# BradenDKelly/MetropolisMonteCarlo

Measured on AMD Instinct MI355X. Metric: MC trial moves/sec (whole node), SPC/E NVT full Ewald fp64, higher is better.
Workload: dtype f64

## Files before the change

### metropolismontecarlo_amd/csrc/mmc_wave.hpp

```cpp
#pragma once
#include "mmc_fast.hpp"
#include "mmc_propose.hpp"

#ifndef WV_WAVES
#define WV_WAVES 4
#endif
#ifndef WV_OCC
#define WV_OCC 5
#endif
#ifndef WV_OCC_WOLF
#define WV_OCC_WOLF 4
#endif
#ifndef WV_MWAVES
#define WV_MWAVES WV_WAVES
#endif
#ifndef WV_LIST
#define WV_LIST 640
#endif
#ifndef WV_PF
#define WV_PF 6
#endif
#define MMC_CQ_PAD (4 * 64 * (2 * WV_PF + 2))
#ifndef WV_TPF
#define WV_TPF 3
#endif

typedef uint16_t wv_list_t;
#define MMC_WAVE_MAX_MOL 65535
template <int NW, bool PT = true> struct WaveSharedT {
    alignas(16) double qtab[MMC_QQ_TABLE_DOUBLES];
    cplx ptab[NW][2][3][3][MMC_NKTAB];
    wv_list_t list[NW][WV_LIST];
    alignas(16) double pvw[NW][12];
    alignas(16) double outw[NW][8];
    __device__ __forceinline__ double *sum6w(int wv) { return reinterpret_cast<double *>(&ptab[wv][0][0][0][0]); }
};
template <int NW> struct WaveSharedT<NW, false> {
    alignas(16) double qtab[MMC_QQ_TABLE_DOUBLES];
    alignas(16) double sum6[NW][24];
    wv_list_t list[NW][WV_LIST];
    alignas(16) double pvw[NW][12];
    alignas(16) double outw[NW][8];
    __device__ __forceinline__ double *sum6w(int wv) { return sum6[wv]; }
};
typedef WaveSharedT<WV_WAVES> WaveShared;

#ifdef WV_STAMPS
#define WV_NSTAMP 8
__device__ unsigned long long g_wv_stamps[65536 * WV_NSTAMP];
#define WV_STAMP(i)                                                                              \
    do {                                                                                         \
        asm volatile("s_waitcnt vmcnt(0) lgkmcnt(0)" ::: "memory");                              \
        if (lane == 0 && unit < 65536)                                                           \
            g_wv_stamps[unit * WV_NSTAMP + (i)] = __builtin_amdgcn_s_memtime();                  \
    } while (0)
#else
#define WV_STAMP(i)
#endif

__device__ __forceinline__ void wave_sync()
{
    __builtin_amdgcn_fence(__ATOMIC_RELEASE, "wavefront");
    __builtin_amdgcn_wave_barrier();
    __builtin_amdgcn_fence(__ATOMIC_ACQUIRE, "wavefront");
}

__device__ __forceinline__ double dpp_quad_swap_f64(double v)
{
    const long long b = __double_as_longlong(v);
    const unsigned lo = (unsigned)__builtin_amdgcn_update_dpp(0, (int)b, 0xB1, 0xf, 0xf, true),
                   hi = (unsigned)__builtin_amdgcn_update_dpp(0, (int)(b >> 32), 0xB1, 0xf, 0xf, true);
    return __longlong_as_double((long long)(((unsigned long long)hi << 32) | lo));
}
__device__ __forceinline__ void wave_sum6_add(double v0, double v1, double v2, double v3, double v4,
                                              double v5, double *out, double *scratch, int lane)
{
    const bool odd = (lane & 1) != 0;
    double p0 = (odd ? v1 : v0) + dpp_quad_swap_f64(odd ? v0 : v1);
    double p1 = (odd ? v3 : v2) + dpp_quad_swap_f64(odd ? v2 : v3);
    double p2 = (odd ? v5 : v4) + dpp_quad_swap_f64(odd ? v4 : v5);
    p0 += dpp_row_shr_f64<2>(p0); p1 += dpp_row_shr_f64<2>(p1); p2 += dpp_row_shr_f64<2>(p2);
    p0 += dpp_row_shr_f64<4>(p0); p1 += dpp_row_shr_f64<4>(p1); p2 += dpp_row_shr_f64<4>(p2);
    p0 += dpp_row_shr_f64<8>(p0); p1 += dpp_row_shr_f64<8>(p1); p2 += dpp_row_shr_f64<8>(p2);
    if ((lane & 14) == 14) {
        double *dst = scratch + 4 * (lane & 1) + (lane >> 4);
        dst[0] = p0; dst[8] = p1; dst[16] = p2;
    }
    __builtin_amdgcn_fence(__ATOMIC_RELEASE, "wavefront");
    __builtin_amdgcn_wave_barrier();
    __builtin_amdgcn_fence(__ATOMIC_ACQUIRE, "wavefront");
    if (lane < 6) {
        const double *r = scratch + 4 * lane;
        out[lane] += ((r[0] + r[1]) + r[2]) + r[3];
    }
}
__device__ __forceinline__ void wave_sum4_add(double v0, double v1, double v4, double v5, double *out,
                                              double *scratch, int lane)
{
    const bool odd = (lane & 1) != 0;
    double p0 = (odd ? v1 : v0) + dpp_quad_swap_f64(odd ? v0 : v1);
    double p1 = (odd ? v5 : v4) + dpp_quad_swap_f64(odd ? v4 : v5);
    p0 += dpp_row_shr_f64<2>(p0); p1 += dpp_row_shr_f64<2>(p1);
    p0 += dpp_row_shr_f64<4>(p0); p1 += dpp_row_shr_f64<4>(p1);
    p0 += dpp_row_shr_f64<8>(p0); p1 += dpp_row_shr_f64<8>(p1);
    if ((lane & 14) == 14) {
        double *dst = scratch + 4 * (lane & 1) + (lane >> 4);
        dst[0] = p0; dst[8] = p1;
    }
    __builtin_amdgcn_fence(__ATOMIC_RELEASE, "wavefront");
    __builtin_amdgcn_wave_barrier();
    __builtin_amdgcn_fence(__ATOMIC_ACQUIRE, "wavefront");
    if (lane < 4) {
        const double *r = scratch + 4 * lane;
        out[lane < 2 ? lane : lane + 2] += ((r[0] + r[1]) + r[2]) + r[3];
    }
}
__device__ __forceinline__ void wave_sum1_store(double v, double *out, double *scratch, int lane)
{
    v += dpp_row_shr_f64<1>(v);
    v += dpp_row_shr_f64<2>(v);
    v += dpp_row_shr_f64<4>(v);
    v += dpp_row_shr_f64<8>(v);
    if ((lane & 15) == 15)
        scratch[lane >> 4] = v;
    __builtin_amdgcn_fence(__ATOMIC_RELEASE, "wavefront");
    __builtin_amdgcn_wave_barrier();
    __builtin_amdgcn_fence(__ATOMIC_ACQUIRE, "wavefront");
    if (lane == 0)
        *out = ((scratch[0] + scratch[1]) + scratch[2]) + scratch[3];
}

__device__ __forceinline__ int lane_i32(int v, int src)
{
    return __builtin_amdgcn_readlane(v, src);
}

__device__ __forceinline__ double uniform_f64(double v)
{
    const long long b = __double_as_longlong(v);
    unsigned lo, hi;
    asm volatile("v_readfirstlane_b32 %0, %1" : "=s"(lo) : "v"((int)b));
    asm volatile("v_readfirstlane_b32 %0, %1" : "=s"(hi) : "v"((int)(b >> 32)));
    return __longlong_as_double((long long)(((unsigned long long)hi << 32) | lo));
}

__device__ __forceinline__ double lane_f64(double v, int src)
{
    const long long b = __double_as_longlong(v);
    const unsigned lo = (unsigned)__builtin_amdgcn_readlane((int)b, src);
    const unsigned hi = (unsigned)__builtin_amdgcn_readlane((int)(b >> 32), src);
    return __longlong_as_double((long long)(((unsigned long long)hi << 32) | lo));
}

__device__ __forceinline__ void phase_row_moderate(double x, double L, cplx *row )
{
    double sn, cs;
    sincos_moderate(MMC_TWOPI * x / L, sn, cs);
    const cplx e1 = { cs, sn }, one = { 1.0, 0.0 };
    row[5] = one;
    row[6] = e1;
    row[4] = c_conj(e1);
    cplx p = e1;
#pragma unroll
    for (int k = 2; k <= 5; k++) {
        p = c_mul(p, e1);
        row[5 + k] = p;
        row[5 - k] = c_conj(p);
    }
}

__device__ __forceinline__ int wave_decide(const double *outw, bool ov_old, bool ov_new,
                                           const DecideConsts *__restrict__ dc, long long step, int r,
                                           int scur, int lane, double *delta_out = nullptr, bool store_flags = true,
                                           bool flip_s = true)
{
    const double delta = mmc_move_delta(outw, ov_old, ov_new, dc->factor);
    if (delta_out)
        *delta_out = delta;
    const double x = delta / dc->temperature;
    const double u = mmc_metropolis_uniform(ChainKey{ dc->seed, dc->replica0 + (uint32_t)r }, (uint64_t)step);
    bool met;
    if (x < 0.0) met = true;
    else if (1.0 - x > u + 1e-9) met = true;
    else if ((1.0 + x) * u > 1.0 + 1e-9) met = false;
    else met = exp(-x) > u;
    const int acc = (met && !(ov_old || ov_new)) ? 1 : 0;
    if (store_flags && lane == 0)
        dc->flags[r] = (uint8_t)(acc | ((scur ^ (flip_s ? acc : 0)) << 1));
    return acc;
}

__device__ __forceinline__ int wave_ticket(unsigned *queue, unsigned base, int n_waves, int lane)
{
    unsigned t = 0;
    if (lane == 0)
        t = atomicAdd(queue, 1u);
    return n_waves + (int)(__builtin_amdgcn_readfirstlane(t) - base);
}

template <bool SUBST, bool IMG, bool MULTI = false, bool WOLF = false>
__global__ __launch_bounds__(WV_MWAVES * 64)
__attribute__((amdgpu_waves_per_eu(WOLF ? WV_OCC_WOLF : WV_OCC, WOLF ? WV_OCC_WOLF : WV_OCC))) void k_move_eval_wave(
    BatchView bv, double *rec, const double *__restrict__ qq_tab,
    const int32_t *__restrict__ kpack, FastConsts fc, const MoveRec *__restrict__ cur,
    const MoveRec *__restrict__ prev, PartOut *out, int n_parts, PairParams pp, int r_base,
    int n_units, const uint8_t *flagv, unsigned stamp, const DecideConsts *__restrict__ dc, long long dec_step,
    int n_sub_arg, int slot0, unsigned *queue, unsigned queue_base)
{
    const int n_sub = MULTI ? n_sub_arg : 1;
    __shared__ __align__(16) WaveSharedT<WV_MWAVES, !WOLF> sm;
    const int tid = threadIdx.x, lane0 = tid & 63;
    const int wv = __builtin_amdgcn_readfirstlane(tid >> 6);

    for (int k = tid; k < MMC_QQ_TABLE_DOUBLES; k += WV_MWAVES * 64)
        sm.qtab[k] = qq_tab[k];
    __syncthreads();

    const int n_mol = bv.n_mol, nkv = bv.nkvecs;
    const double box = bv.box;
    const BoxConsts bc = box_consts(box);
    const int np = WOLF ? n_parts : (n_parts == 1) ? 1 : n_parts - 1;
    const int plen = (n_mol + np - 1) / np;
    const bool same_gate = pp.lj_gate_sq == pp.qq_gate_sq;
    const double inv_box = uniform_f64(1.0 / box);
    uint32_t gate_q;
    asm volatile("v_readfirstlane_b32 %0, %1" : "=s"(gate_q) : "v"(com_quant_gate(fmax(pp.lj_gate_sq, pp.qq_gate_sq), box)));
    wv_list_t *const list = sm.list[wv];
    const double *const pvw = sm.pvw[wv];

    for (int unit = blockIdx.x * WV_MWAVES + wv; unit < n_units;
         unit = MULTI && queue ? wave_ticket(queue, queue_base, gridDim.x * WV_MWAVES, lane0)
                               : unit + gridDim.x * WV_MWAVES) {
        int lane = lane0;
        if (!MULTI)
            asm volatile("" : "+v"(lane));
        int rl = unit, part = 0;
        if (n_parts != 1) {
            rl = unit / n_parts;
            part = unit - rl * n_parts;
        }
        const int r = r_base + rl;
        const bool do_pairs = WOLF ? true : (n_parts == 1) || (part < n_parts - 1);
        const bool do_recip = WOLF ? false : (n_parts == 1) || (part == n_parts - 1);
        const int j_begin = do_pairs ? min(part * plen, n_mol) : 0;
        const int j_end = do_pairs ? min(j_begin + plen, n_mol) : 0;
        double *const myrec = rec + (int64_t)r * n_mol * MMC_RSTRIDE;

        int flags_carry = -1;
        double e_sum = 0.0;
        unsigned acc_mask = 0, ovl_mask = 0, kind_mask = 0;
      for (int sub = 0; sub < n_sub; sub++) {
        if (MULTI) {
            lane = lane0;
            asm volatile("" : "+v"(lane));
        }
        const MoveRec *cur_s = cur, *prev_s = prev;
        if (n_sub > 1) {
            const int sl = (slot0 + sub) % dc->ring_slots, slp = (slot0 + sub + dc->ring_slots - 1) % dc->ring_slots;
            cur_s = dc->ring + (int64_t)sl * dc->ring_stride;
            if (sub > 0)
                prev_s = dc->ring + (int64_t)slp * dc->ring_stride;
        }
        WV_STAMP(0);
        const double *mvp = reinterpret_cast<const double *>(cur_s + r);
        double w = 0.0;
        if (lane < MV_Q_NEW)
            w = mvp[lane];
        WV_STAMP(1);
        const int gflag = flags_carry >= 0 ? flags_carry : (flagv ? __builtin_amdgcn_readfirstlane((int)flagv[r]) : -1);
        const long long hdr = __double_as_longlong(w);
        const int i0 = lane_i32((int)hdr, 0) - 1;
        const int flags = gflag >= 0 ? gflag : lane_i32((int)(hdr >> 32), 0);
        const bool commit = prev_s && (flags & 1);
        const int scur = (flags >> 1) & 1;

        int pend = -1;
        if (commit) {
            const double *pvp = reinterpret_cast<const double *>(prev_s + r);
            double pw = 0.0;
            if (lane < 9) pw = pvp[MV_AT_NEW + lane];
            else if (lane < 12) pw = pvp[MV_COM_NEW + lane - 9];
            else if (lane == 12) pw = pvp[0];
            else if (lane < 17) pw = pvp[MV_Q_NEW + lane - 13];
            pend = lane_i32((int)__double_as_longlong(pw), 12) - 1;
            if (lane < 12)
                sm.pvw[wv][lane] = pw;
            if (part == 0 && lane < 12) {
                myrec[(int64_t)pend * MMC_RSTRIDE + lane] = pw;
                if (lane < 9) {
                    const int a = lane / 3, d = lane % 3;
                    (d == 0 ? bv.ax : d == 1 ? bv.ay : bv.az)[r * bv.atom_stride + 3 * pend + a] = pw;
                } else {
                    const int d = lane - 9;
                    (d == 0 ? bv.comx : d == 1 ? bv.comy : bv.comz)[r * bv.mol_stride + pend] = pw;
                    comq_store(bv, r, pend, d, pw, inv_box);
                }
            }
            if (bv.quat) {
                const double q0 = wave_pick(pw, 13), q1 = wave_pick(pw, 14),
                             q2 = wave_pick(pw, 15), q3 = wave_pick(pw, 16);
                if (part == 0 && lane >= 13 && lane < 17)
                    quat_commit(bv, r, pend, lane - 13, pw, q0 * q0 + q1 * q1 + q2 * q2 + q3 * q3 > 0.25);
            }
            wave_sync();
            if (WOLF && !SUBST)
                asm volatile("s_waitcnt vmcnt(0)" ::: "memory");
        }

#define WV_CQ_BASE (bv.comq + (int64_t)r * 3 * bv.cq_stride)
#define WV_PART_DST (out + (int64_t)r * n_parts + part)
        auto decide_here = [&](bool o0, bool o1) -> int {
            if (!dc)
                return 0;
            if (n_sub <= 1)
                return wave_decide(sm.outw[wv], o0, o1, dc, dec_step, r, scur, lane, nullptr, true, !WOLF);
            double delta;
            const bool last = sub + 1 == n_sub;
            const int acc = wave_decide(sm.outw[wv], o0, o1, dc, dec_step + sub, r, scur, lane, &delta, last, !WOLF);
            if (acc) {
                e_sum += delta;
                acc_mask |= 1u << sub;
            }
            if (o0 || o1)
                ovl_mask |= 1u << sub;
            kind_mask |= (unsigned)((lane_i32((int)(hdr >> 32), 0) >> 8) & 1) << sub;
            flags_carry = acc | ((scur ^ (WOLF ? 0 : acc)) << 1);
            if (last) {
                wave_sync();
                if (lane < 7)
                    sm.outw[wv][lane] = lane == 0 ? e_sum
                                 : lane == 1 ? __longlong_as_double((long long)acc_mask | ((long long)ovl_mask << 32))
                                 : lane == 2 ? __longlong_as_double((long long)kind_mask) : 0.0;
                wave_sync();
            }
            return acc;
        };
#define WV_DECIDE(o0, o1) decide_here(o0, o1)
#define WV_RECORD_OVL(o) (n_sub > 1 ? false : (o))
#define WV_STORE_IF (sub + 1 == n_sub)
#define WV_STORE_SYSTEM MULTI
#define WV_ZERO opaque_f64(0.0)
#define WV_SUBST SUBST
#define WV_IMG IMG
#define WV_WOLF WOLF
#define WV_VIRIAL (!MULTI)
#ifndef WV_XY_MOVE
#define WV_XY_MOVE 1
#endif
#define WV_XY WV_XY_MOVE
#define WV_PASSES 2
#define WV_AFTER_PHASE_TABLES                                                                    \
    if (!SUBST && commit)                                                                        \
        asm volatile("s_waitcnt vmcnt(0)" ::: "memory");
#include "mmc_wave_unit.inc"
#undef WV_AFTER_PHASE_TABLES
#undef WV_IMG
#undef WV_WOLF
#undef WV_VIRIAL
#undef WV_PASSES
#undef WV_XY
#undef WV_SUBST
#undef WV_ZERO
#undef WV_CQ_BASE
#undef WV_PART_DST
#undef WV_DECIDE
#undef WV_RECORD_OVL
#undef WV_STORE_IF
#undef WV_STORE_SYSTEM
        if (n_sub > 1)
            asm volatile("s_waitcnt vmcnt(0)" ::: "memory");
      }
    }
}

struct TotalWaveShared {
    alignas(16) double qtab[MMC_QQ_TABLE_DOUBLES];
    int32_t list[WV_WAVES][WV_LIST];
};

#define WV_TOTAL_WAVES_PER_SIMD 5
template <bool COHERENT, bool IMG>
__device__ __forceinline__ void total_wave_body(
    TotalWaveShared &sm, const BatchView &bv, const double *__restrict__ rec,
    const double *__restrict__ qq_tab, const FastConsts &fc, const PairParams &pp, TotalPart *out,
    int units_per_rep, int n_units, int paired, int wg, int n_wgs, int j_chunk = 0)
{
    const int tid = threadIdx.x, lane0 = tid & 63;
    const int wv = __builtin_amdgcn_readfirstlane(tid >> 6);
    for (int k = tid; k < MMC_QQ_TABLE_DOUBLES; k += WV_WAVES * 64)
        sm.qtab[k] = qq_tab[k];
    __syncthreads();

    const int n_mol = bv.n_mol;
    const double box = bv.box;
    const BoxConsts bc = box_consts(box);
    const bool same_gate = pp.lj_gate_sq == pp.qq_gate_sq;
    const double inv_box = 1.0 / box;
    const uint32_t gate_q = com_quant_gate(fmax(pp.lj_gate_sq, pp.qq_gate_sq), box);
    int32_t *const list = sm.list[wv];

    for (int unit = wg * WV_WAVES + wv; unit < n_units; unit += n_wgs * WV_WAVES) {
        int lane = lane0;
        asm volatile("" : "+v"(lane));
        const int r = unit / units_per_rep, u = unit - r * units_per_rep;
        const double *myrec = rec + (int64_t)r * n_mol * MMC_RSTRIDE;
        const uint16_t *cq0 = bv.comq + (int64_t)r * 3 * bv.cq_stride;
        const uint32_t *sxy = reinterpret_cast<const uint32_t *>(cq0);
        const uint16_t *sz = cq0 + 2 * bv.cq_stride;
        double a_lj = 0, a_v = 0, a_q = 0;
        unsigned long long ovm = 0;

        const int n_ch = j_chunk > 0 ? (n_mol + j_chunk - 1) / j_chunk : 1;
        const int j_lo = j_chunk > 0 ? (u % n_ch) * j_chunk : 0;
        const int j_hi = j_chunk > 0 ? min(j_lo + j_chunk, n_mol) : n_mol;
        const int iA = j_chunk > 0 ? u / n_ch : u, iB = n_mol - 1 - u;
        const bool hasB = paired && iB > iA;
        double wAB = 0.0;
        if (lane < MMC_REC)
            wAB = myrec[(int64_t)iA * MMC_RSTRIDE + lane];
        else if (hasB && lane >= 16 && lane < 16 + MMC_REC)
            wAB = myrec[(int64_t)iB * MMC_RSTRIDE + lane - 16];

        auto process = [&](int cnt) {
            wave_sync();
            for (int n0 = 0; n0 < cnt; n0 += 64) {
                const int n = n0 + lane;
                const bool act = n < cnt;
                const int ent = act ? list[n] : 0;
                const int j = ent & ((1 << 27) - 1);
                const bool isB = (ent >> 27) != 0;
                double t[MMC_REC];
                const double2 *src = reinterpret_cast<const double2 *>(myrec + (int64_t)j * MMC_RSTRIDE);
#pragma unroll
                for (int q = 0; q < 6; q++) {
                    const double2 v = src[q];
                    t[2 * q] = v.x;
                    t[2 * q + 1] = v.y;
                }
                const int own0 = isB ? 16 : 0;
                auto mine = [&](int word) { return wave_pick(wAB, own0 + word); };
                const double ccx = mine(9), ccy = mine(10), ccz = mine(11);
                double m[3] = { 0, 0, 0 };
                auto min1 = [&](int d, double a, double b) {
                    if constexpr (IMG)
                        return fma(m[d], bc.neg, b - a);
                    else
                        return vector1D_abs(a, b, bc);
                };
                if constexpr (IMG) {
                    const double dx = t[9] - ccx, dy = t[10] - ccy, dz = t[11] - ccz;
                    m[0] = (fabs(dx) < bc.half) ? 0.0 : copysign(1.0, dx);
                    m[1] = (fabs(dy) < bc.half) ? 0.0 : copysign(1.0, dy);
                    m[2] = (fabs(dz) < bc.half) ? 0.0 : copysign(1.0, dz);
                }
                const double x0 = min1(0, ccx, t[9]), y0 = min1(1, ccy, t[10]), z0 = min1(2, ccz, t[11]);
                const double c0 = x0 * x0 + y0 * y0 + z0 * z0;
                const bool g0 = act && (c0 < pp.qq_gate_sq);
                const bool l0 = same_gate ? g0 : (act && (c0 < pp.lj_gate_sq));
                const unsigned long long gm0 = wave_ballot(g0);
                auto pair_ab = [&](int ab, double ax, double ay, double az, double bx, double by,
                                   double bz) {
                    const double qq = fc.qq9[ab];
                    const bool qneg = (fc.qneg_mask >> ab) & 1;
                    const double px = min1(0, ax, bx), py = min1(1, ay, by), pz = min1(2, az, bz);
                    const double u0 = px * px + py * py + pz * pz;
                    const unsigned long long cm0 = wave_ballot(u0 < pp.ovr) & gm0;
                    const unsigned long long im0 = (IMG ? ~0ULL : wave_ballot(u0 < pp.qq_slack_sq)) & (qneg ? gm0 & ~cm0 : gm0);
                    double e0 = qq_table_eval_lanes(sm.qtab, u0, im0);
                    if (qneg) {
                        ovm |= cm0;
                    } else if (cm0 != 0ULL) {
                        if (((im0 >> lane) & 1) && u0 < MMC_QQ_UMIN) e0 = qq_pair_cold(u0, pp.kappa);
                    }
                    a_q = fma(e0, qq, a_q);
                    const double eps = fc.eps9[ab], sg = fc.sig9[ab];
                    if ((fc.lj_mask >> ab) & 1) {
                        if (l0 && (IMG || u0 < pp.lj_slack_sq)) {
                            const double s2 = sg * sg / u0;
                            const double s6 = s2 * s2 * s2;
                            const double s12 = s6 * s6;
                            const double virab = eps * (2.0 * s12 - s6);
                            const double f0 = (IMG ? px : vector1D(ax, bx, bc)) * virab * s2,
                                         f1 = (IMG ? py : vector1D(ay, by, bc)) * virab * s2,
                                         f2 = (IMG ? pz : vector1D(az, bz, bc)) * virab * s2;
                            a_lj += eps * (s12 - s6);
                            a_v += (IMG ? x0 : vector1D(ccx, t[9], bc)) * f0 + (IMG ? y0 : vector1D(ccy, t[10], bc)) * f1
                                   + (IMG ? z0 : vector1D(ccz, t[11], bc)) * f2;
                        }
                    }
                };
#pragma unroll 1
                for (int a = 0; a < 3; a++) {
                    const double ax = mine(3 * a), ay = mine(3 * a + 1), az = mine(3 * a + 2);
                    pair_ab(3 * a, ax, ay, az, t[0], t[1], t[2]);
                    __builtin_amdgcn_sched_barrier(0);
                    pair_ab(3 * a + 1, ax, ay, az, t[3], t[4], t[5]);
                    __builtin_amdgcn_sched_barrier(0);
                    pair_ab(3 * a + 2, ax, ay, az, t[6], t[7], t[8]);
                    __builtin_amdgcn_sched_barrier(0);
                }
            }
            wave_sync();
        };

        int cnt = 0;
        for (int half = 0; half < (hasB ? 2 : 1); half++) {
            const int i0 = half == 0 ? iA : iB;
            const int woff = half == 0 ? 0 : 16;
            uint32_t cqxy, cqz;
            {
                const int t = lane & 15;
                const int myq = (t >= 9 && t < 12) ? (int)com_quant(wAB, inv_box) : 0;
                cqxy = (uint32_t)lane_i32(myq, woff + 9) | (uint32_t)lane_i32(myq, woff + 10) << 16;
                cqz = (uint32_t)lane_i32(myq, woff + 11);
            }
            const int first = max(i0 + 1, j_lo);
            int base = first & ~63;
            const char *pxy = reinterpret_cast<const char *>(sxy) + 4 * (int64_t)base;
            const char *pz = reinterpret_cast<const char *>(sz) + 2 * (int64_t)base;
            const uint32_t ul4 = 4u * (uint32_t)lane, ul2 = 2u * (uint32_t)lane;
            uint32_t fxy[WV_TPF], fz[WV_TPF];
#pragma unroll
            for (int b = 0; b < WV_TPF; b++) {
                fxy[b] = *reinterpret_cast<const uint32_t *>(pxy + 256 * b + ul4);
                fz[b] = *reinterpret_cast<const uint16_t *>(pz + 128 * b + ul2);
            }
            while (base < j_hi) {
#pragma unroll
                for (int b = 0; b < WV_TPF; b++) {
                    const int j = base + lane;
                    const uint32_t xy = fxy[b], z = fz[b];
                    fxy[b] = *reinterpret_cast<const uint32_t *>(pxy + 256 * (b + WV_TPF) + ul4);
                    fz[b] = *reinterpret_cast<const uint16_t *>(pz + 128 * (b + WV_TPF) + ul2);
                    const bool keep = (com_quant_dist2(xy, z, cqxy, cqz) < gate_q)
                                      && ((uint32_t)(j - first) < (uint32_t)(j_hi - first));
                    const unsigned long long m = wave_ballot(keep);
                    if (keep)
                        list[cnt + lanes_below(m)] = j | (half << 27);
                    cnt += __popcll(m);
                    base += 64;
                }
                pxy += 256 * WV_TPF;
                pz += 128 * WV_TPF;
                if (cnt > WV_LIST - 64 * WV_TPF) {
                    process(cnt);
                    cnt = 0;
                }
            }
        }
        if (cnt)
            process(cnt);
        const double s0 = wave_sum_rows(a_lj), s1 = wave_sum_rows(a_v), s2 = wave_sum_rows(a_q);
        const bool any_ovl = ovm != 0ULL;
        if (lane == 0) {
            TotalPart o;
            o.lj_pot = s0; o.lj_vir = s1; o.qq = s2;
            o.n_ovl = any_ovl ? 1 : 0;
            o._pad = 0;
            if (COHERENT) {
                double *w = reinterpret_cast<double *>(out + unit);
                __hip_atomic_store(w, o.lj_pot, __ATOMIC_RELAXED, __HIP_MEMORY_SCOPE_AGENT);
                __hip_atomic_store(w + 1, o.lj_vir, __ATOMIC_RELAXED, __HIP_MEMORY_SCOPE_AGENT);
                __hip_atomic_store(w + 2, o.qq, __ATOMIC_RELAXED, __HIP_MEMORY_SCOPE_AGENT);
                __hip_atomic_store(reinterpret_cast<long long *>(w + 3), (long long)o.n_ovl,
                                   __ATOMIC_RELAXED, __HIP_MEMORY_SCOPE_AGENT);
            } else {
                out[unit] = o;
            }
        }
    }
}

template <bool IMG>
__global__ __launch_bounds__(WV_WAVES * 64, WV_TOTAL_WAVES_PER_SIMD) void k_total_wave(
    BatchView bv, const double *__restrict__ rec, const double *__restrict__ qq_tab, FastConsts fc,
    PairParams pp, TotalPart *out, int units_per_rep, int n_units, int paired)
{
    __shared__ __align__(16) TotalWaveShared sm;
    total_wave_body<false, IMG>(sm, bv, rec, qq_tab, fc, pp, out, units_per_rep, n_units, paired,
                           (int)blockIdx.x, (int)gridDim.x);
}

__global__ __launch_bounds__(MMC_BLOCK) void k_total_reduce(const TotalPart *parts, int n_parts,
                                                             TotalsRaw *out)
{
    __shared__ double red[4 * MMC_WAVES];
    const int r = blockIdx.x;
    const TotalPart *p = parts + (int64_t)r * n_parts;
    double v[4] = { 0, 0, 0, 0 }, tot[4];
    for (int k = threadIdx.x; k < n_parts; k += MMC_BLOCK) {
        v[0] += p[k].lj_pot; v[1] += p[k].lj_vir; v[2] += p[k].qq; v[3] += (double)p[k].n_ovl;
    }
    block_sum<4>(v, red, tot);
    if (threadIdx.x == 0) {
        TotalsRaw t;
        t.lj_e = 2.0 * (tot[0] * 4);
        t.lj_v = 2.0 * (tot[1] * 24 / 3.0);
        t.qq = 2.0 * tot[2];
        t.n_ovl = tot[3] > 0 ? 1 : 0;
        t._pad = 0;
        out[r] = t;
    }
}

#define SRV_WAVES 8
struct ServerArgs {
    const unsigned long long *ctrl;
    const double2 *steps;
    uint64_t seed, replica0;
    int64_t rng_off;
    int32_t *timeout_flag;
    uint64_t seq_off;
};
#define SRV_ACCEPT 1u
#define SRV_SCUR 2u
#define SRV_STEPS 4u
#define SRV_QUIT 8u
#define SRV_TIMEOUT_TICKS 300000000ULL
#define SRV_GAVE_UP (~0ULL)

__global__ __launch_bounds__(SRV_WAVES * 64, 2) void k_move_server_wave(
    BatchView bv, double *rec, const double *__restrict__ qq_tab,
    const int32_t *__restrict__ kpack, FastConsts fc, PartOut *out, int n_parts, PairParams pp,
    ServerArgs sa)
{
    __shared__ __align__(16) WaveSharedT<SRV_WAVES> sm;
    __shared__ __align__(16) double mvw_all[SRV_WAVES][32];
    __shared__ __align__(16) double comb[8];
    __shared__ unsigned long long ctl;
    const int tid = threadIdx.x;
    int lane = tid & 63;
    const int wv = __builtin_amdgcn_readfirstlane(tid >> 6);
    for (int k = tid; k < MMC_QQ_TABLE_DOUBLES; k += blockDim.x)
        sm.qtab[k] = qq_tab[k];
    __syncthreads();

    const int n_mol = bv.n_mol, nkv = bv.nkvecs;
    const double box = bv.box;
    const BoxConsts bc = box_consts(box);
    const int np = n_parts - 1;
    const int plen = (n_mol + np - 1) / np;
    const bool same_gate = pp.lj_gate_sq == pp.qq_gate_sq;
    const double inv_box = 1.0 / box;
    const uint32_t gate_q = com_quant_gate(fmax(pp.lj_gate_sq, pp.qq_gate_sq), box);
    wv_list_t *const list = sm.list[wv];
    const double *const pvw = sm.pvw[wv];
    double *const mvw = mvw_all[wv];

    const int r = blockIdx.x, part = wv;
    const int unit = r * n_parts + part;
    (void)unit;
    const bool do_pairs = part < n_parts - 1;
    const bool do_recip = part == n_parts - 1;
    const int j_begin = do_pairs ? min(part * plen, n_mol) : 0;
    const int j_end = do_pairs ? min(j_begin + plen, n_mol) : 0;
    double *const myrec = rec + (int64_t)r * n_mol * MMC_RSTRIDE;
    const uint16_t *const cq_base = bv.comq + (int64_t)r * 3 * bv.cq_stride;
// ... 158 lines not shown
```

### metropolismontecarlo_amd/csrc/mmc_wave_unit.inc

```
#ifndef WV_NS
#define WV_NS 2
#define WV_NS_DEFAULTED
#endif
#if WV_NS == 2
#define WV_IF2(...) __VA_ARGS__
#else
#define WV_IF2(...)
#endif
#ifndef WV_SUBST
#define WV_SUBST 1
#define WV_SUBST_DEFAULTED
#endif
#ifndef WV_IMG
#define WV_IMG 0
#define WV_IMG_DEFAULTED
#endif
#ifndef WV_PASSES
#define WV_PASSES 1
#define WV_PASSES_DEFAULTED
#endif
#ifndef WV_XY
#define WV_XY 0
#define WV_XY_DEFAULTED
#endif
#ifndef WV_KPF
#define WV_KPF 2
#endif
#ifndef WV_WOLF
#define WV_WOLF 0
#define WV_WOLF_DEFAULTED
#endif
#ifndef WV_ZERO
#define WV_ZERO 0.0
#define WV_ZERO_DEFAULTED
#endif
#ifndef WV_VIRIAL
#define WV_VIRIAL 1
#define WV_VIRIAL_DEFAULTED
#endif
#ifndef WV_STORE_IF
#define WV_STORE_IF true
#define WV_STORE_IF_DEFAULTED
#endif
#if WV_NS != 2
static_assert(WV_VIRIAL, "the one-state body always delivers the virial");
#endif
        double *const outw = sm.outw[wv];
        unsigned long long ovm0 = 0, ovm1 = 0;

        constexpr bool wv_wolf = WV_WOLF;
        if constexpr (!wv_wolf) {
        if (do_recip) {
            {
                const int t = lane < 18 ? lane : 0;
                const int st = t / 9, q = t - 9 * st;
                const double x = wave_pick(w, (st ? MV_AT_NEW : MV_AT_OLD) + q);
                if (lane < 18)
                    phase_row_moderate(x, box, sm.ptab[wv][st][q / 3][q % 3]);
            }
            wave_sync();
            WV_STAMP(2);
#ifdef WV_AFTER_PHASE_TABLES
            WV_AFTER_PHASE_TABLES
#endif
        }
        auto recip_loop = [&]() {
            double a_rec = 0;
#ifdef WV_S_BASE
            const double *So = WV_S_BASE;
            double *Sn = WV_S_DST;
#else
            const double *So = s_buf(bv, r, scur);
            double *Sn = s_buf(bv, r, scur ^ 1);
#endif
            int kcs[WV_KPF], kps[WV_KPF];
            double cfs[WV_KPF];
            double2 sos[WV_KPF];
#pragma unroll
            for (int q = 0; q < WV_KPF; q++) {
                kcs[q] = min(lane + 64 * q, nkv - 1);
                kps[q] = kpack[kcs[q]];
                cfs[q] = bv.cfac[kcs[q]];
                sos[q] = *reinterpret_cast<const double2 *>(So + 2 * kcs[q]);
            }
#if WV_XY
            const int colp = kpack[MMC_NK_STRIDE + lane];
#endif
#if WV_XY
            cplx xyp[2][3];
            {
                const int cx = colp & 15, cy = (colp >> 4) & 15;
#pragma unroll
                for (int st = 0; st < 2; st++)
#pragma unroll
                    for (int l = 0; l < 3; l++)
                        xyp[st][l] = c_mul_fused(sm.ptab[wv][st][l][0][5 + cx], sm.ptab[wv][st][l][1][cy]);
            }
#endif
#ifdef WV_S_MIRROR
            unsigned long long s_sum = 0;
#endif
            const int n_it = (nkv + 63) >> 6;
            int k = lane;
            for (int it = 0; it < n_it; it++) {
                const int kc = kcs[0], kp = kps[0];
                const double cf = cfs[0];
                const double2 so = sos[0];
#pragma unroll
                for (int q = 0; q + 1 < WV_KPF; q++) {
                    kcs[q] = kcs[q + 1]; kps[q] = kps[q + 1]; cfs[q] = cfs[q + 1]; sos[q] = sos[q + 1];
                }
                kcs[WV_KPF - 1] = min(k + 64 * WV_KPF, nkv - 1);
                kps[WV_KPF - 1] = kpack[kcs[WV_KPF - 1]];
                cfs[WV_KPF - 1] = bv.cfac[kcs[WV_KPF - 1]];
                sos[WV_KPF - 1] = *reinterpret_cast<const double2 *>(So + 2 * kcs[WV_KPF - 1]);
                {
                    const int kz = (kp >> 8) & 15;
                    double nr = so.x, ni = so.y;
#if WV_XY
                    const int col = (kp >> 12) & (MMC_KCOLS - 1);
                    auto from_col = [&](const cplx &v) {
                        cplx o;
                        o.re = wave_pick(v.re, col);
                        o.im = wave_pick(v.im, col);
                        return o;
                    };
#else
                    const int kx = kp & 15, ky = (kp >> 4) & 15;
#endif
#pragma unroll
                    for (int l = 0; l < 3; l++) {
#if WV_XY
                        const cplx tn = c_mul_fused(from_col(xyp[1][l]), sm.ptab[wv][1][l][2][kz]);
                        const cplx to = c_mul_fused(from_col(xyp[0][l]), sm.ptab[wv][0][l][2][kz]);
#else
                        const cplx tn = c_mul_fused(c_mul_fused(sm.ptab[wv][1][l][0][5 + kx], sm.ptab[wv][1][l][1][ky]),
                                                sm.ptab[wv][1][l][2][kz]);
                        const cplx to = c_mul_fused(c_mul_fused(sm.ptab[wv][0][l][0][5 + kx], sm.ptab[wv][0][l][1][ky]),
                                                sm.ptab[wv][0][l][2][kz]);
#endif
                        nr = fma(fc.q[l], tn.re - to.re, nr);
                        ni = fma(fc.q[l], tn.im - to.im, ni);
                    }
                    *reinterpret_cast<double2 *>(Sn + 2 * kc) = make_double2(nr, ni);
#ifdef WV_S_MIRROR
                    {
                        typedef double s_piece __attribute__((ext_vector_type(2)));
                        s_piece v;
                        v.x = nr; v.y = ni;
                        double *mp = WV_S_MIRROR + 2 * kc;
                        asm volatile("global_store_dwordx4 %0, %1, off sc0 sc1" ::"v"(mp), "v"(v) : "memory");
                        if (k < nkv)
                            s_sum += (unsigned long long)__double_as_longlong(nr)
                                     + 3ULL * (unsigned long long)__double_as_longlong(ni);
                    }
#endif
                    const double wgt = k < nkv ? cf : 0.0;
                    a_rec = fma(wgt, fma(nr, nr, ni * ni) - fma(so.x, so.x, so.y * so.y), a_rec);
                }
                k += 64;
            }
            wave_sum1_store(a_rec, &outw[6], outw, lane);
#ifdef WV_S_MIRROR
            s_sum = wave_sum_u64(s_sum);
            if (lane == 0)
                sm.pvw[wv][0] = __longlong_as_double((long long)s_sum);
#endif
            WV_STAMP(3);
            wave_sync();
        };
        if (do_recip)
            recip_loop();
        }
        if (!do_recip && lane == 0)
            outw[6] = WV_ZERO;

        if (do_pairs) {
            if (lane < 6)
                outw[lane] = WV_ZERO;
            double cc[2][3];
            uint32_t cqxy[2], cqz[2];
            {
                const bool is_com = WV_IF2((lane >= MV_COM_OLD && lane < MV_COM_OLD + 3) ||)
                                    (lane >= MV_COM_NEW && lane < MV_COM_NEW + 3);
                const int myq = is_com ? (int)com_quant(w, inv_box) : 0;
#pragma unroll
                for (int d = 0; d < 3; d++) {
                    WV_IF2(cc[0][d] = lane_f64(w, MV_COM_OLD + d);)
                    cc[1][d] = lane_f64(w, MV_COM_NEW + d);
                }
                WV_IF2(cqxy[0] = (uint32_t)lane_i32(myq, MV_COM_OLD) | (uint32_t)lane_i32(myq, MV_COM_OLD + 1) << 16;)
                cqxy[1] = (uint32_t)lane_i32(myq, MV_COM_NEW) | (uint32_t)lane_i32(myq, MV_COM_NEW + 1) << 16;
                WV_IF2(cqz[0] = (uint32_t)lane_i32(myq, MV_COM_OLD + 2);)
                cqz[1] = (uint32_t)lane_i32(myq, MV_COM_NEW + 2);
            }

            auto process = [&](int cnt) {
                WV_IF2(double a_lj0 = 0, a_v0 = 0, a_q0 = 0;)
                double a_lj1 = 0, a_v1 = 0, a_q1 = 0;
                wave_sync();
                for (int n0 = 0; n0 < cnt; n0 += 64) {
                    const int n = n0 + lane;
                    const int j = n < cnt ? list[n] : 0;
                    const bool act = (n < cnt) && (j != i0);
                    double t[MMC_REC];
                    const double2 *src = reinterpret_cast<const double2 *>(myrec + (int64_t)j * MMC_RSTRIDE);
#pragma unroll
                    for (int q = 0; q < 6; q++) {
                        const double2 v = src[q];
                        t[2 * q] = v.x;
                        t[2 * q + 1] = v.y;
                    }
                    if (n0 == 0)
                        WV_STAMP(5);
                    if (WV_SUBST && j == pend) {
#pragma unroll
                        for (int q = 0; q < MMC_REC; q++)
                            t[q] = pvw[q];
                    }
                    WV_IF2(bool g0, l0;)
                    bool g1, l1;
                    constexpr bool wv_img = WV_IMG;
                    constexpr bool wv_virial = WV_VIRIAL;
                    double m[2][3] = { { 0, 0, 0 }, { 0, 0, 0 } };
                    auto min1 = [&](int st, int d, double a, double b) {
                        if constexpr (wv_img)
                            return fma(m[st][d], bc.neg, b - a);
                        else
                            return vector1D_abs(a, b, bc);
                    };
#define WV_MIN1(st, d, a, b) min1(st, d, a, b)
                    {
                        if constexpr (wv_img) {
#pragma unroll
                            for (int d = 0; d < 3; d++) {
                                const double d1 = t[9 + d] - cc[1][d];
                                m[1][d] = (fabs(d1) < bc.half) ? 0.0 : copysign(1.0, d1);
#if WV_NS == 2
                                const double d0 = t[9 + d] - cc[0][d];
                                m[0][d] = (fabs(d0) < bc.half) ? 0.0 : copysign(1.0, d0);
#endif
                            }
                        }
#if WV_NS == 2
                        const double x0 = WV_MIN1(0, 0, cc[0][0], t[9]), y0 = WV_MIN1(0, 1, cc[0][1], t[10]),
                                     z0 = WV_MIN1(0, 2, cc[0][2], t[11]);
                        const double c0 = x0 * x0 + y0 * y0 + z0 * z0;
                        g0 = act && (c0 < pp.qq_gate_sq);
                        l0 = same_gate ? g0 : (act && (c0 < pp.lj_gate_sq));
#endif
                        const double x1 = WV_MIN1(1, 0, cc[1][0], t[9]), y1 = WV_MIN1(1, 1, cc[1][1], t[10]),
                                     z1 = WV_MIN1(1, 2, cc[1][2], t[11]);
                        const double c1 = x1 * x1 + y1 * y1 + z1 * z1;
                        g1 = act && (c1 < pp.qq_gate_sq);
                        l1 = same_gate ? g1 : (act && (c1 < pp.lj_gate_sq));
                    }
                    WV_IF2(const unsigned long long gm0 = wave_ballot(g0);)
                    const unsigned long long gm1 = wave_ballot(g1);
#if WV_PASSES == 2
#define WV_PAIR_FENCE
                    auto pass = [&](auto stc, bool g, bool l, unsigned long long gm, unsigned long long &ovm,
                                    double &a_lj, double &a_v, double &a_q) {
                        constexpr int ST = decltype(stc)::value;
#pragma unroll 1
                        for (int a = 0; a < 3; a++) {
                            const int base_w = (ST ? MV_AT_NEW : MV_AT_OLD) + 3 * a;
                            const double ax = lane_f64(w, base_w), ay = lane_f64(w, base_w + 1),
                                         az = lane_f64(w, base_w + 2);
                            auto pair1 = [&](int ab, double bx, double by, double bz) {
                                const double qq = fc.qq9[ab];
                                const bool qneg = (fc.qneg_mask >> ab) & 1;
                                const double px = WV_MIN1(ST, 0, ax, bx), py = WV_MIN1(ST, 1, ay, by),
                                             pz = WV_MIN1(ST, 2, az, bz);
                                const double u = px * px + py * py + pz * pz;
                                const unsigned long long cm = wave_ballot(u < pp.ovr) & gm;
                                const unsigned long long qm = qneg ? cm : 0ULL, cold = cm & ~qm;
                                const unsigned long long im = (wv_img ? ~0ULL : wave_ballot(u < pp.qq_slack_sq)) & gm & ~qm;
                                double e = qq_table_eval_lanes(sm.qtab, u, im);
                                ovm |= qm;
                                if (cold != 0ULL) {
                                    if (((im >> lane) & 1) && u < MMC_QQ_UMIN) e = qq_pair_cold(u, pp.kappa);
                                }
                                a_q = fma(e, qq, a_q);
                                if ((fc.lj_mask >> ab) & 1) {
                                    const double eps = fc.eps9[ab], sg = fc.sig9[ab];
                                    if (l && (wv_img || u < pp.lj_slack_sq)) {
                                        const double s2 = sg * sg / u;
                                        const double s6 = s2 * s2 * s2;
                                        const double s12 = s6 * s6;
                                        double f0, f1, f2;
                                        if constexpr (wv_virial) {
                                            const double virab = eps * (2.0 * s12 - s6);
                                            f0 = (wv_img ? px : vector1D(ax, bx, bc)) * virab * s2;
                                            f1 = (wv_img ? py : vector1D(ay, by, bc)) * virab * s2;
                                            f2 = (wv_img ? pz : vector1D(az, bz, bc)) * virab * s2;
                                        }
                                        a_lj += eps * (s12 - s6);
                                        if constexpr (wv_virial) {
                                            a_v += (wv_img ? WV_MIN1(ST, 0, cc[ST][0], t[9]) : vector1D(cc[ST][0], t[9], bc)) * f0
                                                   + (wv_img ? WV_MIN1(ST, 1, cc[ST][1], t[10]) : vector1D(cc[ST][1], t[10], bc)) * f1
                                                   + (wv_img ? WV_MIN1(ST, 2, cc[ST][2], t[11]) : vector1D(cc[ST][2], t[11], bc)) * f2;
                                        }
                                    }
                                }
                            };
                            pair1(3 * a, t[0], t[1], t[2]);
                            WV_PAIR_FENCE
                            pair1(3 * a + 1, t[3], t[4], t[5]);
                            WV_PAIR_FENCE
                            pair1(3 * a + 2, t[6], t[7], t[8]);
                            WV_PAIR_FENCE
                        }
                        (void)g;
                    };
                    WV_IF2(pass(std::integral_constant<int, 0>{}, g0, l0, gm0, ovm0, a_lj0, a_v0, a_q0);)
                    pass(std::integral_constant<int, 1>{}, g1, l1, gm1, ovm1, a_lj1, a_v1, a_q1);
                }
#else
                    auto pair_ab = [&](int ab, double a0x, double a0y, double a0z, double a1x,
                                       double a1y, double a1z, double bx, double by, double bz) {
                        const double qq = fc.qq9[ab];
                        const bool qneg = (fc.qneg_mask >> ab) & 1;
#if WV_NS == 2
                        const double p0x = WV_MIN1(0, 0, a0x, bx), p0y = WV_MIN1(0, 1, a0y, by),
                                     p0z = WV_MIN1(0, 2, a0z, bz);
                        const double u0 = p0x * p0x + p0y * p0y + p0z * p0z;
                        const unsigned long long cm0 = wave_ballot(u0 < pp.ovr) & gm0;
                        const unsigned long long im0 = wave_ballot(u0 < pp.qq_slack_sq) & (qneg ? gm0 & ~cm0 : gm0);
                        double e0 = qq_table_eval_lanes(sm.qtab, u0, im0);
#else
                        (void)a0x; (void)a0y; (void)a0z;
#endif
                        const double p1x = WV_MIN1(1, 0, a1x, bx), p1y = WV_MIN1(1, 1, a1y, by),
                                     p1z = WV_MIN1(1, 2, a1z, bz);
                        const double u1 = p1x * p1x + p1y * p1y + p1z * p1z;
                        const unsigned long long cm1 = wave_ballot(u1 < pp.ovr) & gm1;
                        const unsigned long long im1 = wave_ballot(u1 < pp.qq_slack_sq) & (qneg ? gm1 & ~cm1 : gm1);
                        double e1 = qq_table_eval_lanes(sm.qtab, u1, im1);
                        if (qneg) {
                            WV_IF2(ovm0 |= cm0;)
                            ovm1 |= cm1;
                        } else if ((WV_IF2(cm0 |) cm1) != 0ULL) {
                            WV_IF2(if (((im0 >> lane) & 1) && u0 < MMC_QQ_UMIN) e0 = qq_pair_cold(u0, pp.kappa);)
                            if (((im1 >> lane) & 1) && u1 < MMC_QQ_UMIN) e1 = qq_pair_cold(u1, pp.kappa);
                        }
                        WV_IF2(a_q0 = fma(e0, qq, a_q0);)
                        a_q1 = fma(e1, qq, a_q1);
                        const double eps = fc.eps9[ab], sg = fc.sig9[ab];
                        if ((fc.lj_mask >> ab) & 1) {
#if WV_NS == 2
                            if (l0 && u0 < pp.lj_slack_sq) {
                                const double s2 = sg * sg / u0;
                                const double s6 = s2 * s2 * s2;
                                const double s12 = s6 * s6;
                                double f0, f1, f2;
                                if constexpr (wv_virial) {
                                    const double virab = eps * (2.0 * s12 - s6);
                                    f0 = (wv_img ? p0x : vector1D(a0x, bx, bc)) * virab * s2;
                                    f1 = (wv_img ? p0y : vector1D(a0y, by, bc)) * virab * s2;
                                    f2 = (wv_img ? p0z : vector1D(a0z, bz, bc)) * virab * s2;
                                }
                                a_lj0 += eps * (s12 - s6);
                                if constexpr (wv_virial) {
                                    a_v0 += (wv_img ? WV_MIN1(0, 0, cc[0][0], t[9]) : vector1D(cc[0][0], t[9], bc)) * f0
                                            + (wv_img ? WV_MIN1(0, 1, cc[0][1], t[10]) : vector1D(cc[0][1], t[10], bc)) * f1
                                            + (wv_img ? WV_MIN1(0, 2, cc[0][2], t[11]) : vector1D(cc[0][2], t[11], bc)) * f2;
                                }
                            }
#endif
                            if (l1 && u1 < pp.lj_slack_sq) {
                                const double s2 = sg * sg / u1;
                                const double s6 = s2 * s2 * s2;
                                const double s12 = s6 * s6;
                                double f0, f1, f2;
                                if constexpr (wv_virial) {
                                    const double virab = eps * (2.0 * s12 - s6);
                                    f0 = (wv_img ? p1x : vector1D(a1x, bx, bc)) * virab * s2;
                                    f1 = (wv_img ? p1y : vector1D(a1y, by, bc)) * virab * s2;
                                    f2 = (wv_img ? p1z : vector1D(a1z, bz, bc)) * virab * s2;
                                }
                                a_lj1 += eps * (s12 - s6);
                                if constexpr (wv_virial) {
                                    a_v1 += (wv_img ? WV_MIN1(1, 0, cc[1][0], t[9]) : vector1D(cc[1][0], t[9], bc)) * f0
                                            + (wv_img ? WV_MIN1(1, 1, cc[1][1], t[10]) : vector1D(cc[1][1], t[10], bc)) * f1
                                            + (wv_img ? WV_MIN1(1, 2, cc[1][2], t[11]) : vector1D(cc[1][2], t[11], bc)) * f2;
                                }
                            }
                        }
                    };
#pragma unroll 1
                    for (int a = 0; a < 3; a++) {
#if WV_NS == 2
                        const double a0x = lane_f64(w, MV_AT_OLD + 3 * a),
                                     a0y = lane_f64(w, MV_AT_OLD + 3 * a + 1),
                                     a0z = lane_f64(w, MV_AT_OLD + 3 * a + 2);
#else
                        const double a0x = 0.0, a0y = 0.0, a0z = 0.0;
#endif
                        const double a1x = lane_f64(w, MV_AT_NEW + 3 * a),
                                     a1y = lane_f64(w, MV_AT_NEW + 3 * a + 1),
                                     a1z = lane_f64(w, MV_AT_NEW + 3 * a + 2);
                        pair_ab(3 * a, a0x, a0y, a0z, a1x, a1y, a1z, t[0], t[1], t[2]);
                        __builtin_amdgcn_sched_barrier(0);
                        pair_ab(3 * a + 1, a0x, a0y, a0z, a1x, a1y, a1z, t[3], t[4], t[5]);
                        __builtin_amdgcn_sched_barrier(0);
                        pair_ab(3 * a + 2, a0x, a0y, a0z, a1x, a1y, a1z, t[6], t[7], t[8]);
                        __builtin_amdgcn_sched_barrier(0);
                    }
                }
#endif
#undef WV_MIN1
#if WV_NS == 2
                if constexpr (WV_VIRIAL)
                    wave_sum6_add(a_lj0, a_lj1, a_v0, a_v1, a_q0, a_q1, outw, sm.sum6w(wv), lane);
                else
                    wave_sum4_add(a_lj0, a_lj1, a_q0, a_q1, outw, sm.sum6w(wv), lane);
#else
                const double s1 = wave_sum_rows(a_lj1), s3 = wave_sum_rows(a_v1), s5 = wave_sum_rows(a_q1);
                if (lane == 0) {
                    outw[1] += s1; outw[3] += s3; outw[5] += s5;
                }
#endif
                wave_sync();
            };

            const char *pxy = reinterpret_cast<const char *>(WV_CQ_BASE) + 4 * (int64_t)j_begin;
            const char *pz = reinterpret_cast<const char *>(WV_CQ_BASE + 2 * bv.cq_stride) + 2 * (int64_t)j_begin;
            const uint32_t ul4 = 4u * (uint32_t)lane, ul2 = 2u * (uint32_t)lane;
            uint32_t pqxy = 0, pqz = 0;
            if (WV_SUBST && pend >= 0) {
                pqxy = (uint32_t)__builtin_amdgcn_readfirstlane((int)com_quant(pvw[9], inv_box))
                       | (uint32_t)__builtin_amdgcn_readfirstlane((int)com_quant(pvw[10], inv_box)) << 16;
                pqz = (uint32_t)__builtin_amdgcn_readfirstlane((int)com_quant(pvw[11], inv_box));
            }
            int base = j_begin, cnt = 0;
            uint32_t fxy[WV_PF], fz[WV_PF];
#pragma unroll
            for (int b = 0; b < WV_PF; b++) {
                fxy[b] = *reinterpret_cast<const uint32_t *>(pxy + 256 * b + ul4);
                fz[b] = *reinterpret_cast<const uint16_t *>(pz + 128 * b + ul2);
            }
            while (base < j_end) {
#pragma unroll
                for (int b = 0; b < WV_PF; b++) {
                    const int j = base + lane;
                    uint32_t xy = fxy[b], z = fz[b];
                    fxy[b] = *reinterpret_cast<const uint32_t *>(pxy + 256 * (b + WV_PF) + ul4);
                    fz[b] = *reinterpret_cast<const uint16_t *>(pz + 128 * (b + WV_PF) + ul2);
                    if (WV_SUBST && j == pend) { xy = pqxy; z = pqz; }
                    const bool keep = WV_IF2((com_quant_dist2(xy, z, cqxy[0], cqz[0]) < gate_q) |)
                                      (com_quant_dist2(xy, z, cqxy[1], cqz[1]) < gate_q);
                    const int nv = j_end - base;
                    const unsigned long long m_end = nv >= 64 ? ~0ULL : (nv > 0 ? (1ULL << nv) - 1ULL : 0ULL);
                    const unsigned long long m = wave_ballot(keep);
                    if (keep)
                        list[cnt + lanes_below(m)] = j;
                    cnt += __popcll(m & m_end);
                    base += 64;
                }
                pxy += 256 * WV_PF;
                pz += 128 * WV_PF;
                if (cnt > WV_LIST - 64 * WV_PF) {
                    process(cnt);
                    cnt = 0;
                }
            }
            WV_STAMP(4);
            if (cnt)
                process(cnt);
            WV_STAMP(6);
        } else if (lane < 6) {
            outw[lane] = WV_ZERO;
        }
#ifdef WV_S_MIRROR
        if (do_recip && !do_pairs) {
            wave_sync();
            if (lane == 0)
                outw[0] = sm.pvw[wv][0];
        }
#endif

#ifdef WV_UNIT_NO_STORE
        if (lane == 0)
            outw[7] = __longlong_as_double((long long)((ovm0 != 0ULL ? 1 : 0) | (ovm1 != 0ULL ? 2 : 0)));
#else
        wave_sync();
        {
#ifdef WV_DECIDE
            const int accept = WV_DECIDE(ovm0 != 0ULL, ovm1 != 0ULL);
#else
            const int accept = 0;
#endif
            if (WV_STORE_IF) {
                const uint32_t csum = part_checksum_lanes(lane < 7 ? outw[lane] : 0.0, lane, stamp);
#ifdef WV_RECORD_OVL
                if (lane == 0)
                    outw[7] = pack_ovl(WV_RECORD_OVL(ovm0 != 0ULL), WV_RECORD_OVL(ovm1 != 0ULL), stamp, csum, accept);
#else
                if (lane == 0)
                    outw[7] = pack_ovl(ovm0 != 0ULL, ovm1 != 0ULL, stamp, csum, accept);
#endif
            }
        }
        wave_sync();
#ifdef WV_STORE_WT
        store_part<true>(WV_PART_DST, sm.outw[wv], lane);
#else
#ifndef WV_STORE_SYSTEM
#define WV_STORE_SYSTEM false
#define WV_STORE_SYSTEM_DEFAULTED
#endif
        if (WV_STORE_IF)
            store_part<WV_STORE_SYSTEM>(WV_PART_DST, sm.outw[wv], lane);
#ifdef WV_STORE_SYSTEM_DEFAULTED
#undef WV_STORE_SYSTEM
#undef WV_STORE_SYSTEM_DEFAULTED
#endif
#endif
        wave_sync();
        WV_STAMP(7);
#endif
#ifdef WV_STORE_IF_DEFAULTED
#undef WV_STORE_IF
#undef WV_STORE_IF_DEFAULTED
#endif
#undef WV_IF2
#ifdef WV_XY_DEFAULTED
#undef WV_XY
#undef WV_XY_DEFAULTED
#endif
#ifdef WV_PASSES_DEFAULTED
#undef WV_PASSES
#undef WV_PASSES_DEFAULTED
#endif
#ifdef WV_IMG_DEFAULTED
#undef WV_IMG
#undef WV_IMG_DEFAULTED
#endif
#ifdef WV_SUBST_DEFAULTED
#undef WV_SUBST
#undef WV_SUBST_DEFAULTED
#endif
#ifdef WV_ZERO_DEFAULTED
#undef WV_ZERO
#undef WV_ZERO_DEFAULTED
#endif
#ifdef WV_VIRIAL_DEFAULTED
#undef WV_VIRIAL
#undef WV_VIRIAL_DEFAULTED
#endif
#ifdef WV_WOLF_DEFAULTED
#undef WV_WOLF
#undef WV_WOLF_DEFAULTED
#endif
#ifdef WV_NS_DEFAULTED
#undef WV_NS
#undef WV_NS_DEFAULTED
#endif
```

Before: 150.1 million.

## Prefetch next sub-step move record and carry commit data in registers

In multi-substep mode, the next ring slot's move record is loaded early, just before the wave sums, so its latency overlaps the reduction. The committed previous move is taken from the registers that already hold it rather than re-read from global memory when there is no quaternion and a single part. The pair loop also hoists the per-atom charge and LJ parameters into scalar registers, and the neighbour-list build loop is restructured so the prefetch buffer is reloaded after each flush. The added register state and control flow may raise register pressure and affect occupancy.

```diff
diff --git a/metropolismontecarlo_amd/csrc/mmc_wave.hpp b/metropolismontecarlo_amd/csrc/mmc_wave.hpp
--- a/metropolismontecarlo_amd/csrc/mmc_wave.hpp
+++ b/metropolismontecarlo_amd/csrc/mmc_wave.hpp
@@ -249,39 +249,50 @@
         int flags_carry = -1;
         double e_sum = 0.0;
         unsigned acc_mask = 0, ovl_mask = 0, kind_mask = 0;
+        double w = 0.0, w_next = 0.0;
       for (int sub = 0; sub < n_sub; sub++) {
         if (MULTI) {
             lane = lane0;
             asm volatile("" : "+v"(lane));
         }
+        const bool carried = MULTI && sub > 0;
+        const bool commit_from_w = carried && !bv.quat && n_parts == 1;
         const MoveRec *cur_s = cur, *prev_s = prev;
-        if (n_sub > 1) {
-            const int sl = (slot0 + sub) % dc->ring_slots, slp = (slot0 + sub + dc->ring_slots - 1) % dc->ring_slots;
-            cur_s = dc->ring + (int64_t)sl * dc->ring_stride;
-            if (sub > 0)
-                prev_s = dc->ring + (int64_t)slp * dc->ring_stride;
+        if (n_sub > 1 && !carried)
+            cur_s = dc->ring + (int64_t)((slot0 + sub) % dc->ring_slots) * dc->ring_stride;
+        if (carried && !commit_from_w)
+            prev_s = dc->ring + (int64_t)((slot0 + sub + dc->ring_slots - 1) % dc->ring_slots) * dc->ring_stride;
+        WV_STAMP(0);
+        const double w_prev = w;
+        if (carried) {
+            w = w_next;
+        } else {
+            const double *mvp = reinterpret_cast<const double *>(cur_s + r);
+            w = 0.0;
+            if (lane < MV_Q_NEW)
+                w = mvp[lane];
         }
-        WV_STAMP(0);
-        const double *mvp = reinterpret_cast<const double *>(cur_s + r);
-        double w = 0.0;
-        if (lane < MV_Q_NEW)
-            w = mvp[lane];
         WV_STAMP(1);
         const int gflag = flags_carry >= 0 ? flags_carry : (flagv ? __builtin_amdgcn_readfirstlane((int)flagv[r]) : -1);
         const long long hdr = __double_as_longlong(w);
         const int i0 = lane_i32((int)hdr, 0) - 1;
         const int flags = gflag >= 0 ? gflag : lane_i32((int)(hdr >> 32), 0);
-        const bool commit = prev_s && (flags & 1);
+        const bool commit = (commit_from_w || prev_s) && (flags & 1);
         const int scur = (flags >> 1) & 1;
 
         int pend = -1;
         if (commit) {
-            const double *pvp = reinterpret_cast<const double *>(prev_s + r);
             double pw = 0.0;
-            if (lane < 9) pw = pvp[MV_AT_NEW + lane];
-            else if (lane < 12) pw = pvp[MV_COM_NEW + lane - 9];
-            else if (lane == 12) pw = pvp[0];
-            else if (lane < 17) pw = pvp[MV_Q_NEW + lane - 13];
+            if (commit_from_w) {
+                const int src = lane < 9 ? MV_AT_NEW + lane : lane < 12 ? MV_COM_NEW + lane - 9 : 0;
+                pw = wave_pick(w_prev, src);
+            } else {
+                const double *pvp = reinterpret_cast<const double *>(prev_s + r);
+                if (lane < 9) pw = pvp[MV_AT_NEW + lane];
+                else if (lane < 12) pw = pvp[MV_COM_NEW + lane - 9];
+                else if (lane == 12) pw = pvp[0];
+                else if (lane < 17) pw = pvp[MV_Q_NEW + lane - 13];
+            }
             pend = lane_i32((int)__double_as_longlong(pw), 12) - 1;
             if (lane < 12)
                 sm.pvw[wv][lane] = pw;
@@ -352,7 +363,18 @@
 #define WV_AFTER_PHASE_TABLES                                                                    \
     if (!SUBST && commit)                                                                        \
         asm volatile("s_waitcnt vmcnt(0)" ::: "memory");
+        bool next_requested = false;
+#define WV_BEFORE_SUMS                                                                           \
+    if (MULTI && sub + 1 < n_sub && !next_requested) {                                           \
+        const double *nxp = reinterpret_cast<const double *>(                                    \
+            dc->ring + (int64_t)((slot0 + sub + 1) % dc->ring_slots) * dc->ring_stride + r);     \
+        if (lane < MV_Q_NEW)                                                                     \
+            w_next = nxp[lane];                                                                  \
+        next_requested = true;                                                                   \
+    }
 #include "mmc_wave_unit.inc"
+        WV_BEFORE_SUMS
+#undef WV_BEFORE_SUMS
 #undef WV_AFTER_PHASE_TABLES
 #undef WV_IMG
 #undef WV_WOLF
diff --git a/metropolismontecarlo_amd/csrc/mmc_wave_unit.inc b/metropolismontecarlo_amd/csrc/mmc_wave_unit.inc
--- a/metropolismontecarlo_amd/csrc/mmc_wave_unit.inc
+++ b/metropolismontecarlo_amd/csrc/mmc_wave_unit.inc
@@ -264,11 +264,25 @@
                         constexpr int ST = decltype(stc)::value;
 #pragma unroll 1
                         for (int a = 0; a < 3; a++) {
+                            double qq3[3] = { fc.qq9[3 * a], fc.qq9[3 * a + 1], fc.qq9[3 * a + 2] };
+                            double eps3[3] = { 0.0, 0.0, 0.0 }, sig3[3] = { 0.0, 0.0, 0.0 };
+                            const unsigned lj3 = ((unsigned)fc.lj_mask >> (3 * a)) & 7u;
+                            if (lj3 != 0u) {
+#pragma unroll
+                                for (int b = 0; b < 3; b++) {
+                                    eps3[b] = fc.eps9[3 * a + b];
+                                    sig3[b] = fc.sig9[3 * a + b];
+                                }
+                                asm volatile("" : "+s"(eps3[0]), "+s"(eps3[1]), "+s"(eps3[2]),
+                                                  "+s"(sig3[0]), "+s"(sig3[1]), "+s"(sig3[2]));
+                            }
+                            asm volatile("" : "+s"(qq3[0]), "+s"(qq3[1]), "+s"(qq3[2]));
                             const int base_w = (ST ? MV_AT_NEW : MV_AT_OLD) + 3 * a;
                             const double ax = lane_f64(w, base_w), ay = lane_f64(w, base_w + 1),
                                          az = lane_f64(w, base_w + 2);
-                            auto pair1 = [&](int ab, double bx, double by, double bz) {
-                                const double qq = fc.qq9[ab];
+                            auto pair1 = [&](int b, double bx, double by, double bz) {
+                                const int ab = 3 * a + b;
+                                const double qq = qq3[b];
                                 const bool qneg = (fc.qneg_mask >> ab) & 1;
                                 const double px = WV_MIN1(ST, 0, ax, bx), py = WV_MIN1(ST, 1, ay, by),
                                              pz = WV_MIN1(ST, 2, az, bz);
@@ -282,8 +296,8 @@
                                     if (((im >> lane) & 1) && u < MMC_QQ_UMIN) e = qq_pair_cold(u, pp.kappa);
                                 }
                                 a_q = fma(e, qq, a_q);
-                                if ((fc.lj_mask >> ab) & 1) {
-                                    const double eps = fc.eps9[ab], sg = fc.sig9[ab];
+                                if ((lj3 >> b) & 1) {
+                                    const double eps = eps3[b], sg = sig3[b];
                                     if (l && (wv_img || u < pp.lj_slack_sq)) {
                                         const double s2 = sg * sg / u;
                                         const double s6 = s2 * s2 * s2;
@@ -304,11 +318,11 @@
                                     }
                                 }
                             };
-                            pair1(3 * a, t[0], t[1], t[2]);
+                            pair1(0, t[0], t[1], t[2]);
                             WV_PAIR_FENCE
-                            pair1(3 * a + 1, t[3], t[4], t[5]);
+                            pair1(1, t[3], t[4], t[5]);
                             WV_PAIR_FENCE
-                            pair1(3 * a + 2, t[6], t[7], t[8]);
+                            pair1(2, t[6], t[7], t[8]);
                             WV_PAIR_FENCE
                         }
                         (void)g;
@@ -410,6 +424,9 @@
                 }
 #endif
 #undef WV_MIN1
+#ifdef WV_BEFORE_SUMS
+                WV_BEFORE_SUMS
+#endif
 #if WV_NS == 2
                 if constexpr (WV_VIRIAL)
                     wave_sum6_add(a_lj0, a_lj1, a_v0, a_v1, a_q0, a_q1, outw, sm.sum6w(wv), lane);
@@ -433,41 +450,41 @@
                        | (uint32_t)__builtin_amdgcn_readfirstlane((int)com_quant(pvw[10], inv_box)) << 16;
                 pqz = (uint32_t)__builtin_amdgcn_readfirstlane((int)com_quant(pvw[11], inv_box));
             }
-            int base = j_begin, cnt = 0;
-            uint32_t fxy[WV_PF], fz[WV_PF];
-#pragma unroll
-            for (int b = 0; b < WV_PF; b++) {
-                fxy[b] = *reinterpret_cast<const uint32_t *>(pxy + 256 * b + ul4);
-                fz[b] = *reinterpret_cast<const uint16_t *>(pz + 128 * b + ul2);
-            }
-            while (base < j_end) {
+            int base = j_begin, cnt;
+            do {
+                cnt = 0;
+                uint32_t fxy[WV_PF], fz[WV_PF];
 #pragma unroll
                 for (int b = 0; b < WV_PF; b++) {
-                    const int j = base + lane;
-                    uint32_t xy = fxy[b], z = fz[b];
-                    fxy[b] = *reinterpret_cast<const uint32_t *>(pxy + 256 * (b + WV_PF) + ul4);
-                    fz[b] = *reinterpret_cast<const uint16_t *>(pz + 128 * (b + WV_PF) + ul2);
-                    if (WV_SUBST && j == pend) { xy = pqxy; z = pqz; }
-                    const bool keep = WV_IF2((com_quant_dist2(xy, z, cqxy[0], cqz[0]) < gate_q) |)
-                                      (com_quant_dist2(xy, z, cqxy[1], cqz[1]) < gate_q);
-                    const int nv = j_end - base;
-                    const unsigned long long m_end = nv >= 64 ? ~0ULL : (nv > 0 ? (1ULL << nv) - 1ULL : 0ULL);
-                    const unsigned long long m = wave_ballot(keep);
-                    if (keep)
-                        list[cnt + lanes_below(m)] = j;
-                    cnt += __popcll(m & m_end);
-                    base += 64;
-                }
-                pxy += 256 * WV_PF;
-                pz += 128 * WV_PF;
-                if (cnt > WV_LIST - 64 * WV_PF) {
+                    fxy[b] = *reinterpret_cast<const uint32_t *>(pxy + 256 * b + ul4);
+                    fz[b] = *reinterpret_cast<const uint16_t *>(pz + 128 * b + ul2);
+                }
+                while (base < j_end && cnt <= WV_LIST - 64 * WV_PF) {
+#pragma unroll
+                    for (int b = 0; b < WV_PF; b++) {
+                        const int j = base + lane;
+                        uint32_t xy = fxy[b], z = fz[b];
+                        fxy[b] = *reinterpret_cast<const uint32_t *>(pxy + 256 * (b + WV_PF) + ul4);
+                        fz[b] = *reinterpret_cast<const uint16_t *>(pz + 128 * (b + WV_PF) + ul2);
+                        if (WV_SUBST && j == pend) { xy = pqxy; z = pqz; }
+                        const bool keep = WV_IF2((com_quant_dist2(xy, z, cqxy[0], cqz[0]) < gate_q) |)
+                                          (com_quant_dist2(xy, z, cqxy[1], cqz[1]) < gate_q);
+                        const int nv = j_end - base;
+                        const unsigned long long m_end = nv >= 64 ? ~0ULL : (nv > 0 ? (1ULL << nv) - 1ULL : 0ULL);
+                        const unsigned long long m = wave_ballot(keep);
+                        if (keep)
+                            list[cnt + lanes_below(m)] = j;
+                        cnt += __popcll(m & m_end);
+                        base += 64;
+                    }
+                    pxy += 256 * WV_PF;
+                    pz += 128 * WV_PF;
+                }
+                if (base >= j_end)
+                    WV_STAMP(4);
+                if (cnt)
                     process(cnt);
-                    cnt = 0;
-                }
-            }
-            WV_STAMP(4);
-            if (cnt)
-                process(cnt);
+            } while (base < j_end);
             WV_STAMP(6);
         } else if (lane < 6) {
             outw[lane] = WV_ZERO;
```

Result: faster. 154.4 million, median of 6 (+2.8%).
